# qwopqwop200/GPTQ-for-LLaMa

Measured on NVIDIA H100. Metric: tokens/sec LLaMA-7B int4 g128 batch=1; matvec HBM GB/s vs 3.35 TB/s roofline, higher is better.
Workload: dtype f16

## Files before the change

### gptq-for-llama_b200/csrc/decode_mega.cu

```cuda
#include <cuda.h>
#include <cudaTypedefs.h>

#include "common.cuh"
#include "int4_core.cuh"
#include "kernels.h"

namespace gptq {
namespace {

using namespace int4;

constexpr int kTeams = 2;
constexpr int kTeamWarps = 8;
constexpr int kTeamThreads = kTeamWarps * 32;
constexpr int kConsumers = kTeams * kTeamThreads;
constexpr int kConsumerWarps = kTeams * kTeamWarps;
constexpr int kBlock = kConsumers + 32 * kTeams;
constexpr int kSlabCols = 256;
constexpr int kStageSteps = 4;
constexpr int kStepBytes = 4096;
constexpr int kScaleOff = kStageSteps * kStepBytes;
constexpr int kZeroOff = kScaleOff + 512;
constexpr int kStageBytes = 17 * 1024;
constexpr int kHD = 128;
// ... 33 lines not shown
    const int optr_s0 = (ring).stages
#define OPTRACE_END(ring, layer, op)                                                                                   \
    do {                                                                                                               \
        if (g_mega_trace != nullptr && threadIdx.x == 0 && (layer) == 2) {                                              \
            g_mega_trace[blockIdx.x * 64 + 48 + 3 * (op)] = (unsigned long long)(clock64() - optr_t0);                  \
            g_mega_trace[blockIdx.x * 64 + 48 + 3 * (op) + 1] = (unsigned long long)((ring).waited - optr_w0);          \
            g_mega_trace[blockIdx.x * 64 + 48 + 3 * (op) + 2] = (unsigned long long)((ring).stages - optr_s0);          \
        }                                                                                                              \
    } while (0)
#else
#define OPTRACE_BEGIN(ring) \
    do {                    \
    } while (0)
#define OPTRACE_END(ring, layer, op) \
    do {                             \
    } while (0)
#endif

struct MatDesc {
    const __half* sc;
    const uint32_t* qz;
    int gs_steps;
    int tmap;
    int chunk0;
};
struct LayerDesc {
    MatDesc qkv, o, gate, up, down;
    const __half* input_norm;
    const __half* post_norm;
    const int32_t* qkv_perm;
    const int32_t* o_perm;
    const int32_t* mlp_perm;
};
constexpr int kMaxTP = 8;
struct MegaParams {
    int n_layers, H, Hq, I, V, v0, v1, n_heads, max_seq, n_stages, lm_rows;
    int tp_size, tp_rank, tp_exchange;
    float eps, inv_base, scale;
    const __half* embed;
    const __half* final_norm;
    const __half* lm_head;
    const int32_t* tokens;
    const int32_t* positions;
    __half* k_cache;
    __half* v_cache;
    size_t layer_stride;
    __half* logits;
    int32_t* next_token;
    __half* resid[2];
    float* acc_qkv;
    float* acc_o;
    float* acc_g;
    float* acc_u;
    float* acc_d;
    float* part;
    float* rope_cs;
    unsigned long long* bar;
    float* acc_o_loc;
    float* acc_d_loc;
    float* acc_o_peer[kMaxTP];
    float* acc_d_peer[kMaxTP];
    __half* logits_peer[kMaxTP];
    unsigned long long* xbar_peer[kMaxTP];
    LayerDesc layers[kMaxLayers];
    CUtensorMap tmaps[6];
    int batch, xs_stride;
};

__device__ __forceinline__ void team_range(unsigned T, unsigned U, unsigned nb, int& a, int& b) {
    a = (int)((T * U) / nb);
    b = (int)(((T + 1) * U) / nb);
}
struct HeadTeams {
    int first, count;
};
__device__ __forceinline__ HeadTeams head_teams(int head, int n_heads, unsigned nb) {
    const int base = (int)nb / n_heads, rem = (int)nb % n_heads;
    HeadTeams h;
    h.first = head * base + min(head, rem);
    h.count = base + (head < rem ? 1 : 0);
    return h;
}
__device__ __forceinline__ void attn_range(unsigned T, int n_heads, unsigned nb, int upb, int& head, int& b0, int& b1) {
    const int base = (int)nb / n_heads, rem = (int)nb % n_heads;
    const int split = rem * (base + 1);
    int idx, cnt;
    if ((int)T < split) {
        head = (int)T / (base + 1);
        idx = (int)T - head * (base + 1);
        cnt = base + 1;
    } else {
        head = rem + ((int)T - split) / base;
        idx = ((int)T - split) % base;
        cnt = base;
    }
    b0 = idx * upb / cnt;
    b1 = (idx + 1) * upb / cnt;
}

__device__ __forceinline__ int stage_steps(int gpos, int gs_steps, int left) { return min(min(kStageSteps, gs_steps - gpos), left); }

__device__ __forceinline__ int step_pos(const MegaParams& p, int s) { return min(max(p.positions[s], 0), p.max_seq - 1); }

__device__ __forceinline__ HeadTeams seq_teams(const MegaParams& p, int s, unsigned nb) {
    int before = 0, mine = 0, tot = 0;
#pragma unroll 1
    for (int i = 0; i < p.batch; ++i) {
        const int units = step_pos(p, i) / kKeysPerUnit + 1;
        before += i < s ? units : 0;
        mine = i == s ? units : mine;
        tot += units;
    }
    const long long extra = (long long)nb - (long long)p.batch * p.n_heads;
    HeadTeams h;
    h.first = s * p.n_heads + (int)(extra * before / tot);
    h.count = (s + 1) * p.n_heads + (int)(extra * (before + mine) / tot) - h.first;
    return h;
}
__device__ __forceinline__ int team_seq(const MegaParams& p, unsigned T, unsigned nb, HeadTeams& st) {
    int s = 0;
#pragma unroll 1
    for (;; ++s) {
        st = seq_teams(p, s, nb);
        if ((int)T < st.first + st.count || s == p.batch - 1) return s;
    }
}
template <bool BATCH>
__device__ __forceinline__ int attn_work(const MegaParams& p, unsigned T, unsigned nb, int& pos, int& Tlen, int& head, int& b0, int& b1) {
    int s = 0;
    HeadTeams st{0, (int)nb};
    if constexpr (BATCH) s = team_seq(p, T, nb, st);
    pos = step_pos(p, s);
    Tlen = pos + 1;
    const int upb = (Tlen + kKeysPerUnit - 1) / kKeysPerUnit;
    attn_range(T - st.first, p.n_heads, st.count, upb, head, b0, b1);
    return s;
}

__device__ __forceinline__ void team_sync(int team) { asm volatile("bar.sync %0, 256;" ::"r"(team + 1) : "memory"); }
__device__ __forceinline__ void cta_sync() { asm volatile("bar.sync 3, 512;" ::: "memory"); }

struct ProdRing {
    uint32_t ring, full, empty;
    int stage, use, nstages;
#ifdef GPTQ_TRACE
    long long blocked;
#endif
};
__device__ __forceinline__ uint32_t prod_acquire(ProdRing& r, uint32_t& bar) {
#ifdef GPTQ_TRACE
    const long long t0 = clock64();
#endif
    if (r.use > 0) mbar_wait_backoff(r.empty + r.stage * 8, (r.use - 1) & 1u);
#ifdef GPTQ_TRACE
    r.blocked += clock64() - t0;
#endif
    bar = r.full + r.stage * 8;
    return r.ring + r.stage * kStageBytes;
}
__device__ __forceinline__ void prod_advance(ProdRing& r) {
    if (++r.stage == r.nstages) {
        r.stage = 0;
        ++r.use;
    }
}

__device__ __forceinline__ void tma_load_3d(uint32_t dst, const CUtensorMap* tm, int c0, int c1, int c2, uint32_t bar, uint64_t policy) {
    asm volatile("cp.async.bulk.tensor.3d.shared::cluster.global.mbarrier::complete_tx::bytes.L2::cache_hint [%0], [%1, {%2, %3, %4}], [%5], %6;" ::"r"(dst),
                 "l"(tm), "r"(c0), "r"(c1), "r"(c2), "r"(bar), "l"(policy)
                 : "memory");
}

struct StageLoad {
    const CUtensorMap* tm;
    int row, chunk, n;
    const void* a;
    const void* b;
    uint32_t a_off, b_off, a_bytes, b_bytes;
};

template <bool BATCH>
struct StageWalk {
    enum { kQ, kA, kO, kG, kD, kL, kEnd };
    int l = 0, op = -1, u = 0, u1 = 0;
    int Tlen = 0;
    size_t kv = 0;

    __device__ __forceinline__ bool next(const MegaParams& p, unsigned T, unsigned nb, StageLoad& s) {
        while (u >= u1) {
            if (op == kEnd) return false;
            if (++op == kL && l + 1 < p.n_layers) {
                ++l;
                op = kQ;
            }
            if (op == kA) {
                int pos, head;
                const int seq = attn_work<BATCH>(p, T, nb, pos, Tlen, head, u, u1);
                kv = (size_t)l * p.layer_stride + (size_t)(seq * p.n_heads + head) * p.max_seq * kHD;
            } else if (op == kL) {
                team_range(T, (unsigned)((p.v1 - p.v0 + p.lm_rows - 1) / p.lm_rows), nb, u, u1);
            } else if (op != kEnd) {
                int K, N, nm;
                matvec_shape(p, K, N, nm);
                team_range(T, (unsigned)(nm * (N / kSlabCols)) * (K / 32), nb, u, u1);
            }
        }
        s.tm = nullptr;
        s.b = nullptr;
        s.b_bytes = 0;
        if (op == kA) {
            const int nrows = min(kKeysPerUnit, Tlen - u * kKeysPerUnit);
            const size_t off = kv + (size_t)u * kKeysPerUnit * kHD;
            s.a = p.k_cache + off;
            s.b = p.v_cache + off;
            s.a_off = 0;
            s.b_off = kVOff;
            s.a_bytes = s.b_bytes = nrows * 256;
            ++u;
        } else if (op == kL) {
            const int R = p.lm_rows, nrows = min(R, p.v1 - p.v0 - u * R);
            s.a = p.lm_head + (size_t)u * R * p.H;
            s.a_off = 0;
            s.a_bytes = (uint32_t)nrows * p.H * 2;
            ++u;
        } else {
            int K, N, nm;
            matvec_shape(p, K, N, nm);
            const int nk = K / 32, nslab = N / kSlabCols;
            const int slab_v = u / nk, ks = u - slab_v * nk;
            const int mi = slab_v >= nslab ? 1 : 0, slab = slab_v - mi * nslab;
            const LayerDesc& L = p.layers[l];
            const MatDesc& m = op == kQ ? L.qkv : op == kO ? L.o : op == kD ? L.down : mi ? L.up : L.gate;
            const int g = ks / m.gs_steps;
            s.n = stage_steps(ks - g * m.gs_steps, m.gs_steps, min(nk - ks, u1 - u));
            s.tm = &p.tmaps[(s.n == kStageSteps ? 0 : 3) + m.tmap];
            s.row = ks * 4;
            s.chunk = m.chunk0 + slab * (kSlabCols / 32);
            s.a = m.sc + (size_t)g * N + slab * kSlabCols;
            s.b = m.qz + (size_t)g * (N >> 3) + slab * (kSlabCols / 8);
            s.a_off = kScaleOff;
            s.b_off = kZeroOff;
            s.a_bytes = 512;
            s.b_bytes = 128;
            u += s.n;
        }
        return true;
    }

    __device__ __forceinline__ void matvec_shape(const MegaParams& p, int& K, int& N, int& nm) const {
        K = op == kO ? p.Hq : op == kD ? p.I : p.H;
        N = op == kQ ? 3 * p.Hq : op == kG ? p.I : p.H;
        nm = op == kG ? 2 : 1;
    }
};

template <bool BATCH>
__device__ void producer_loop(const MegaParams& p, ProdRing r, unsigned T, unsigned nb) {
    uint64_t policy;
    asm volatile("createpolicy.fractional.L2::evict_first.b64 %0, 1.0;" : "=l"(policy));
    StageWalk<BATCH> walk;
    StageLoad s;
#pragma unroll 1
    while (walk.next(p, T, nb, s)) {
        uint32_t bar;
        const uint32_t dst = prod_acquire(r, bar);
        mbar_expect_tx(bar, (s.tm != nullptr ? s.n * kStepBytes : 0) + s.a_bytes + s.b_bytes);
        if (s.tm != nullptr) {
            if (s.n == kStageSteps) {
                tma_load_3d(dst, s.tm, 0, s.row, s.chunk, bar, policy);
            } else {
                for (int j = 0; j < s.n; ++j) tma_load_3d(dst + j * kStepBytes, s.tm, 0, s.row + 4 * j, s.chunk, bar, policy);
            }
        }
        bulk_copy_g2s(dst + s.a_off, s.a, s.a_bytes, bar, policy);
        if (s.b != nullptr) bulk_copy_g2s(dst + s.b_off, s.b, s.b_bytes, bar, policy);
        prod_advance(r);
    }
#ifdef GPTQ_TRACE
    if (g_mega_trace != nullptr && (T & 1) == 0) g_mega_trace[(T / kTeams) * 64 + 63] = (unsigned long long)r.blocked;
#endif
}

struct ConsRing {
    uint32_t ring, full;
    uint32_t tile, bar;
    uint32_t parity;
    int left, nstages;
#ifdef GPTQ_TRACE
    long long waited;
    int stages;
#endif
};
__device__ __forceinline__ uint32_t cons_wait(ConsRing& c) {
#ifdef GPTQ_TRACE
    const long long t0 = clock64();
#endif
    mbar_wait(c.bar, c.parity);
#ifdef GPTQ_TRACE
    c.waited += clock64() - t0;
    ++c.stages;
#endif
    return c.tile;
}
__device__ __forceinline__ void cons_release(ConsRing& c, int lane) {
    __syncwarp();
    if (lane == 0) mbar_arrive(c.bar + kMaxStages * 8);
    c.tile += kStageBytes;
    c.bar += 8;
    if (--c.left == 0) {
        c.left = c.nstages;
        c.tile = c.ring;
        c.bar = c.full;
        c.parity ^= 1u;
    }
}

__device__ __forceinline__ void grid_barrier(unsigned long long* bar, unsigned long long& target) {
    cta_sync();
    if (threadIdx.x == 0) {
        target += gridDim.x;
        asm volatile("red.release.gpu.global.add.u64 [%0], 1;" ::"l"(bar) : "memory");
        unsigned long long v;
        do {
            asm volatile("ld.acquire.gpu.global.u64 %0, [%1];" : "=l"(v) : "l"(bar) : "memory");
        } while (v < target);
    }
    cta_sync();
}

__device__ __forceinline__ void tp_barrier(const MegaParams& p, unsigned long long& target) {
    cta_sync();
    if (threadIdx.x == 0) {
        target += gridDim.x;
        asm volatile("fence.acq_rel.sys;" ::: "memory");
        for (int q = 0; q < p.tp_size; ++q)
            asm volatile("red.relaxed.sys.global.add.u64 [%0], 1;" ::"l"(p.xbar_peer[q] + 32 * p.tp_rank) : "memory");
        const unsigned long long* mine = p.xbar_peer[p.tp_rank];
        for (int q = 0; q < p.tp_size; ++q) {
            unsigned long long v;
            do {
                asm volatile("ld.relaxed.sys.global.u64 %0, [%1];" : "=l"(v) : "l"(mine + 32 * q) : "memory");
            } while (v < target);
        }
        asm volatile("fence.acq_rel.gpu;" ::: "memory");
    }
    cta_sync();
}

__device__ __forceinline__ void tp_exchange(const MegaParams& p, float* loc, float* const* peers, int n) {
    const int per = (n + gridDim.x - 1) / gridDim.x;
    const int lo = blockIdx.x * per, hi = min(n, lo + per);
    for (int j = lo + threadIdx.x; j < hi; j += kConsumers) {
        const float v = ld_cg(loc + j);
        loc[j] = 0.f;
        for (int q = 0; q < p.tp_size; ++q) asm volatile("red.relaxed.sys.global.add.f32 [%0], %1;" ::"l"(peers[q] + j), "f"(v) : "memory");
    }
}

__device__ __forceinline__ void zero_slice(float* buf, int n) {
    const int per = ((n / 4 + gridDim.x - 1) / gridDim.x);
    const int lo = blockIdx.x * per, hi = min(n / 4, lo + per);
    for (int i = lo + threadIdx.x; i < hi; i += kConsumers) reinterpret_cast<float4*>(buf)[i] = make_float4(0.f, 0.f, 0.f, 0.f);
}

__device__ __forceinline__ float block_sum(float v, uint32_t& m, float* red_s) {
    v = warp_sum(v);
    const uint32_t mx = __reduce_max_sync(0xffffffffu, m & 0xffffu), my = __reduce_max_sync(0xffffffffu, m >> 16);
    cta_sync();
    if ((threadIdx.x & 31) == 0) {
        red_s[threadIdx.x >> 5] = v;
        reinterpret_cast<uint32_t*>(red_s)[kConsumerWarps + (threadIdx.x >> 5)] = mx | (my << 16);
    }
    cta_sync();
    float t = 0.f;
    m = 0;
#pragma unroll
    for (int w = 0; w < kConsumerWarps; ++w) {
        t += red_s[w];
        m = __vmaxu2(m, reinterpret_cast<const uint32_t*>(red_s)[kConsumerWarps + w]);
    }
    return t;
}

__device__ __forceinline__ uint4 perm8(uint32_t w0, uint32_t w1, uint32_t w2, uint32_t w3) {
    return make_uint4(__byte_perm(w0, w2, 0x5410), __byte_perm(w0, w2, 0x7632), __byte_perm(w1, w3, 0x5410), __byte_perm(w1, w3, 0x7632));
}
__device__ __forceinline__ int perm_pos(int j) { return ((j & 3) << 1) + (j >> 2); }

struct XScale {
    float even, odd, inv;
};
__device__ __forceinline__ XScale x_scale(float m) {
    const int e = min(max(14 - ((int)((__float_as_uint(m) >> 23) & 255u) - 127), -1), 38);
    return XScale{__int_as_float((127 + e) << 23), __int_as_float((123 + e) << 23), __int_as_float((127 - e) << 23)};
}
__device__ __forceinline__ uint32_t max_abs8(uint32_t m, uint4 v) {
    m = __vmaxu2(m, v.x & 0x7fff7fffu);
    m = __vmaxu2(m, v.y & 0x7fff7fffu);
    m = __vmaxu2(m, v.z & 0x7fff7fffu);
    return __vmaxu2(m, v.w & 0x7fff7fffu);
}
__device__ __forceinline__ uint32_t scale_h2(uint32_t w, float f) {
    const float2 v = __half22float2(u32_as_h2(w));
    return h2_as_u32(__floats2half2_rn(v.x * f, v.y * f));
}
__device__ __forceinline__ uint4 scale_run(uint4 v, const XScale& sc) {
    return make_uint4(scale_h2(v.x, sc.even), scale_h2(v.y, sc.odd), scale_h2(v.z, sc.even), scale_h2(v.w, sc.odd));
}

__device__ __forceinline__ float run_sum(uint4 v) {
    const float2 a = __half22float2(u32_as_h2(v.x)), b = __half22float2(u32_as_h2(v.y)), c = __half22float2(u32_as_h2(v.z)), d = __half22float2(u32_as_h2(v.w));
    const float even = (a.x + a.y) + (c.x + c.y), odd = (b.x + b.y) + (d.x + d.y);
    return fmaf(odd, 16.0f, even);
}
__device__ __forceinline__ void scale_and_sum(__half* xs, int nsteps, float* xsum, const XScale& sc, int tid, int nthreads) {
    const int n4 = nsteps * 4;
    for (int base = 0; base < n4; base += nthreads) {
        const int idx = base + tid;
        float v = 0.f;
        if (idx < n4) {
            uint4* run = reinterpret_cast<uint4*>(xs + idx * 8);
            const uint4 r = scale_run(*run, sc);
            *run = r;
            v = run_sum(r);
        }
        v += __shfl_xor_sync(0xffffffffu, v, 1);
        v += __shfl_xor_sync(0xffffffffu, v, 2);
        if (idx < n4 && (idx & 3) == 0) xsum[idx >> 2] = v;
    }
}

template <bool ACT, bool PLAIN>
__device__ void stage_norm(const MegaParams& p, const __half* src, const float* acc, const __half* norm_w, __half* resid_out, __half* xs, float* xsum,
                           float* xinv, __half* tmp, float* red_s, const int32_t* perm) {
    const int H = p.H, tid = threadIdx.x, nch = H / 8;
    float ss = 0.f;
    uint32_t xm = 0, wm = 0;
    uint4 nwv[2];
#pragma unroll
    for (int i = 0; i < 2; ++i) {
        const int c = tid + i * kConsumers;
        nwv[i] = make_uint4(0, 0, 0, 0);
        if (c < nch) {
            nwv[i] = *reinterpret_cast<const uint4*>(norm_w + c * 8);
            const uint4 v = ld_cg_u4(src + c * 8);
            uint32_t xv[4] = {v.x, v.y, v.z, v.w};
            if (acc != nullptr) {
                const float4 a0 = ld_cg4(acc + c * 8), a1 = ld_cg4(acc + c * 8 + 4);
                const float av[8] = {a0.x, a0.y, a0.z, a0.w, a1.x, a1.y, a1.z, a1.w};
#pragma unroll
                for (int j = 0; j < 4; ++j)
                    xv[j] = h2_as_u32(__hadd2(u32_as_h2(xv[j]), __floats2half2_rn(av[2 * j], av[2 * j + 1])));
            }
#pragma unroll
            for (int j = 0; j < 4; ++j) {
                const float2 f = __half22float2(u32_as_h2(xv[j]));
                ss = fmaf(f.x, f.x, ss);
                ss = fmaf(f.y, f.y, ss);
            }
            const uint4 xq = make_uint4(xv[0], xv[1], xv[2], xv[3]);
            *reinterpret_cast<uint4*>(tmp + c * 8) = xq;
            xm = max_abs8(xm, xq);
            wm = max_abs8(wm, nwv[i]);
        }
    }
    uint32_t m = max(xm & 0xffffu, xm >> 16) | (max(wm & 0xffffu, wm >> 16) << 16);
    const float tot = block_sum(ss, m, red_s);
    const float rstd = 1.0f / sqrtf(tot / (float)H + p.eps);
    XScale sc{1.f, 1.f, 1.f};
    if constexpr (!PLAIN) {
        sc = x_scale(__half2float(__ushort_as_half((unsigned short)(m & 0xffffu))) * rstd * __half2float(__ushort_as_half((unsigned short)(m >> 16))) * 1.001f);
        if (tid == 0) *xinv = sc.inv;
    }
    if (resid_out != nullptr) {
        const int per = (nch + gridDim.x - 1) / gridDim.x;
        const int c = blockIdx.x * per + tid;
        if (tid < per && c < nch) *reinterpret_cast<uint4*>(resid_out + c * 8) = *reinterpret_cast<const uint4*>(tmp + c * 8);
    }
#pragma unroll
    for (int i = 0; i < 2; ++i) {
        const int c = tid + i * kConsumers;
        if (c < nch) {
            float xf[8];
            bool gathered = false;
            if constexpr (ACT) {
                if (perm != nullptr) {
                    const ::int4 p0 = *reinterpret_cast<const ::int4*>(perm + c * 8), p1 = *reinterpret_cast<const ::int4*>(perm + c * 8 + 4);
                    const int k[8] = {p0.x, p0.y, p0.z, p0.w, p1.x, p1.y, p1.z, p1.w};
#pragma unroll
                    for (int j = 0; j < 8; ++j) xf[j] = __half2float(tmp[k[j]]);
                    gathered = true;
                }
            }
            if (!gathered) {
                const uint4 v = *reinterpret_cast<const uint4*>(tmp + c * 8);
                const uint32_t xv[4] = {v.x, v.y, v.z, v.w};
#pragma unroll
                for (int j = 0; j < 4; ++j) {
                    const float2 f = __half22float2(u32_as_h2(xv[j]));
                    xf[2 * j] = f.x;
                    xf[2 * j + 1] = f.y;
                }
            }
            const uint32_t wv[4] = {nwv[i].x, nwv[i].y, nwv[i].z, nwv[i].w};
            uint32_t o[4];
#pragma unroll
            for (int j = 0; j < 4; ++j) {
                const float2 wf = __half22float2(u32_as_h2(wv[j]));
                o[j] = h2_as_u32(__floats2half2_rn(__fmul_rn(__fmul_rn(xf[2 * j], rstd), wf.x), __fmul_rn(__fmul_rn(xf[2 * j + 1], rstd), wf.y)));
            }
            if constexpr (PLAIN) {
                *reinterpret_cast<uint4*>(xs + c * 8) = make_uint4(o[0], o[1], o[2], o[3]);
            } else {
                const uint4 pv = scale_run(perm8(o[0], o[1], o[2], o[3]), sc);
                *reinterpret_cast<uint4*>(xs + c * 8) = pv;
                float v = run_sum(pv);
                v += __shfl_xor_sync(0xffffffffu, v, 1);
                v += __shfl_xor_sync(0xffffffffu, v, 2);
                if ((c & 3) == 0) xsum[c >> 2] = v;
            }
        }
    }
    cta_sync();
}

__device__ __forceinline__ void mma_16816_z(float (&d)[4], uint32_t a0, uint32_t a1, uint32_t a2, uint32_t a3, uint32_t b0, uint32_t b1) {
    asm volatile("mma.sync.aligned.m16n8k16.row.col.f32.f16.f16.f32 {%0,%1,%2,%3}, {%4,%5,%6,%7}, {%8,%9}, {%10,%10,%10,%10};"
                 : "=f"(d[0]), "=f"(d[1]), "=f"(d[2]), "=f"(d[3])
                 : "r"(a0), "r"(a1), "r"(a2), "r"(a3), "r"(b0), "r"(b1), "f"(0.f));
}

__device__ __forceinline__ void nibble_regs(uint32_t q, uint32_t (&a)[4]) {
    const uint32_t q8 = q >> 8;
    a[0] = q & 0x000f000fu;
    a[1] = q & 0x00f000f0u;
    a[2] = q8 & 0x000f000fu;
    a[3] = q8 & 0x00f000f0u;
}

template <bool FIRST>
__device__ __forceinline__ void step_mma(const uint4& q, const uint4& xf, float (&acc0)[4], float (&acc1)[4]) {
    uint32_t c0[4], c1[4], c2[4], c3[4];
    nibble_regs(q.x, c0);
    nibble_regs(q.y, c1);
    nibble_regs(q.z, c2);
    nibble_regs(q.w, c3);
    if (FIRST) {
        mma_16816_z(acc0, c0[0], c1[0], c0[1], c1[1], xf.x, xf.y);
        mma_16816_z(acc1, c2[0], c3[0], c2[1], c3[1], xf.x, xf.y);
    } else {
        mma_16816(acc0, c0[0], c1[0], c0[1], c1[1], xf.x, xf.y);
        mma_16816(acc1, c2[0], c3[0], c2[1], c3[1], xf.x, xf.y);
    }
    mma_16816(acc0, c0[2], c1[2], c0[3], c1[3], xf.z, xf.w);
    mma_16816(acc1, c2[2], c3[2], c2[3], c3[3], xf.z, xf.w);
}

enum XMode { X_FULL = 0, X_ATTN = 1, X_SWIGLU = 2 };

struct TeamCtx {
    int team, wt, lane, ttid;
    unsigned T, nb;
    __half* xseg;
    float* xsum_seg;
    float* xinv_seg;
    uint32_t* xmax;
    uint8_t* scratch;
};

template <int NB>
__device__ __forceinline__ float merge_records(const MegaParams& p, const HeadTeams& ht, int d) {
    float M = -INFINITY, Ls = 0.f, O = 0.f;
#pragma unroll 1
    for (int ib = 0; ib < ht.count; ib += NB) {
        float mv[NB], lv[NB], ov[NB];
#pragma unroll
        for (int i = 0; i < NB; ++i) {
            const bool on = ib + i < ht.count;
            const float* rc = p.part + (size_t)(ht.first + (on ? ib + i : 0)) * kRec;
            const float m = ld_cg(rc), l = ld_cg(rc + 1), o = ld_cg(rc + 4 + d);
            mv[i] = on ? m : -INFINITY;
            lv[i] = on ? l : 0.f;
            ov[i] = on ? o : 0.f;
        }
        float Mb = M;
#pragma unroll
        for (int i = 0; i < NB; ++i) Mb = fmaxf(Mb, mv[i]);
        const float w0 = (M == -INFINITY) ? 0.f : expf(M - Mb);
        Ls *= w0;
        O *= w0;
#pragma unroll
        for (int i = 0; i < NB; ++i) {
            const float w = (mv[i] == -INFINITY) ? 0.f : expf(mv[i] - Mb);
            Ls = fmaf(lv[i], w, Ls);
            O = fmaf(ov[i], w, O);
        }
        M = Mb;
    }
    return O / Ls;
}

template <int XMODE, bool ACT, bool BATCH>
__device__ void stage_range(const MegaParams& p, const TeamCtx& tc, int nk, int u0, int u1, const int32_t* perm) {
    const int nun = u1 - u0, nfeat = nun * 32;
    const int nbat = BATCH ? p.batch : 1;
    const int ksb = u0 % nk;
    auto k_of = [&](int e) {
        int ks = ksb + (e >> 5);
        if (ks >= nk) ks -= nk;
        return ks * 32 + (e & 31);
    };
    if (tc.ttid < nbat) tc.xmax[tc.ttid] = 0;
    team_sync(tc.team);
    if constexpr (XMODE == X_SWIGLU) {
        for (int c = tc.ttid; c < nun * 4 * nbat; c += kTeamThreads) {
            int s = 0, cs = c;
            if constexpr (BATCH) {
                s = c / (nun * 4);
                cs = c - s * (nun * 4);
            }
            const int k = k_of(cs * 8);
            const float* ag = p.acc_g + (size_t)s * p.I + k;
            const float* au = p.acc_u + (size_t)s * p.I + k;
            const float4 g0 = ld_cg4(ag), g1 = ld_cg4(ag + 4);
            const float4 a0 = ld_cg4(au), a1 = ld_cg4(au + 4);
            const uint32_t o0 = h2_as_u32(__floats2half2_rn(swiglu(g0.x, a0.x), swiglu(g0.y, a0.y)));
            const uint32_t o1 = h2_as_u32(__floats2half2_rn(swiglu(g0.z, a0.z), swiglu(g0.w, a0.w)));
            const uint32_t o2 = h2_as_u32(__floats2half2_rn(swiglu(g1.x, a1.x), swiglu(g1.y, a1.y)));
            const uint32_t o3 = h2_as_u32(__floats2half2_rn(swiglu(g1.z, a1.z), swiglu(g1.w, a1.w)));
            const uint4 pv = perm8(o0, o1, o2, o3);
            *reinterpret_cast<uint4*>(tc.xseg + (size_t)s * p.xs_stride + cs * 8) = pv;
            const uint32_t m = max_abs8(0, pv);
            atomicMax(tc.xmax + s, max(m & 0xffffu, m >> 16));
        }
    } else {
        constexpr int kBatch = 12;
        uint32_t vmax = 0;
        auto put = [&](__half* xseg, int e, float v) {
            const __half hv = __float2half_rn(v);
            xseg[(e & ~7) + perm_pos(e & 7)] = hv;
            vmax = max(vmax, (uint32_t)(__half_as_ushort(hv) & 0x7fffu));
        };
        bool fast = false;
        if constexpr (!BATCH) {
            const int nA = min(nun, nk - ksb);
            const int hA0 = (ksb * 32) / kHD, hA1 = ((ksb + nA) * 32 - 1) / kHD;
            const int nslotA = hA1 - hA0 + 1, nslotB = (nun > nA) ? ((nun - nA) * 32 - 1) / kHD + 1 : 0;
            fast = (nslotA + nslotB <= kTeamWarps) && (nun <= nk) && ((int)tc.nb / p.n_heads + 1 <= kBatch);
            if constexpr (ACT) fast = fast && (perm == nullptr);
            if (fast) {
                float* wts = reinterpret_cast<float*>(tc.scratch);
                float ov[kBatch];
                int slot = 0;
                auto fetch = [&](int e) {
                    const bool active = e < nfeat;
                    const int k = k_of(active ? e : 0);
                    const int head = k / kHD, d = k - head * kHD;
                    slot = ((e >> 5) < nA) ? head - hA0 : nslotA + head;
                    const HeadTeams ht = head_teams(head, p.n_heads, tc.nb);
#pragma unroll
                    for (int i = 0; i < kBatch; ++i) ov[i] = (active && i < ht.count) ? ld_cg(p.part + (size_t)(ht.first + i) * kRec + 4 + d) : 0.f;
                };
                auto emit = [&](int e) {
                    if (e < nfeat) {
                        float O = 0.f;
#pragma unroll
                        for (int i = 0; i < kBatch; ++i) O = fmaf(wts[slot * kBatch + i], ov[i], O);
                        put(tc.xseg, e, O);
                    }
                };
                fetch(tc.ttid);
                if (tc.wt < nslotA + nslotB) {
                    const int lane = tc.lane;
                    const int head = tc.wt < nslotA ? hA0 + tc.wt : tc.wt - nslotA;
                    const HeadTeams ht = head_teams(head, p.n_heads, tc.nb);
                    float m = -INFINITY, l = 0.f;
                    if (lane < ht.count) {
                        m = ld_cg(p.part + (size_t)(ht.first + lane) * kRec);
                        l = ld_cg(p.part + (size_t)(ht.first + lane) * kRec + 1);
                    }
                    float M = m;
#pragma unroll
                    for (int o = 8; o > 0; o >>= 1) M = fmaxf(M, __shfl_xor_sync(0xffffffffu, M, o));
                    M = __shfl_sync(0xffffffffu, M, 0);
                    const float w = (m == -INFINITY) ? 0.f : expf(m - M);
                    float L = l * w;
#pragma unroll
                    for (int o = 8; o > 0; o >>= 1) L += __shfl_xor_sync(0xffffffffu, L, o);
                    L = __shfl_sync(0xffffffffu, L, 0);
                    if (lane < kBatch) wts[tc.wt * kBatch + lane] = w / L;
                }
                team_sync(tc.team);
                emit(tc.ttid);
                for (int e = tc.ttid + kTeamThreads; e - tc.ttid < nfeat; e += kTeamThreads) {
                    fetch(e);
                    emit(e);
                }
                atomicMax(tc.xmax, vmax);
            }
        }
        if (!fast) {
            for (int s = 0; s < nbat; ++s) {
                HeadTeams st{0, (int)tc.nb};
                if constexpr (BATCH) st = seq_teams(p, s, tc.nb);
                for (int e = tc.ttid; e < nfeat; e += kTeamThreads) {
                    int k = k_of(e);
                    if constexpr (ACT) {
                        if (perm != nullptr) k = perm[k];
                    }
                    const int head = k / kHD, d = k - head * kHD;
                    HeadTeams ht = head_teams(head, p.n_heads, st.count);
                    ht.first += st.first;
                    put(tc.xseg + (size_t)s * p.xs_stride, e, merge_records<kBatch>(p, ht, d));
                }
                atomicMax(tc.xmax + s, vmax);
                vmax = 0;
            }
        }
    }
    team_sync(tc.team);
    for (int s = 0; s < nbat; ++s) {
        const XScale sc = x_scale(__half2float(__ushort_as_half((unsigned short)tc.xmax[s])));
        if (tc.ttid == 0) tc.xinv_seg[s] = sc.inv;
        scale_and_sum(tc.xseg + (size_t)s * p.xs_stride, nun, tc.xsum_seg + s * (p.H / 32), sc, tc.ttid, kTeamThreads);
    }
    team_sync(tc.team);
}

template <int NM, int XMODE, bool ACT = false, bool BATCH = false>
__device__ void run_matvec(const MegaParams& p, ConsRing& ring, const TeamCtx& tc, int gs_steps, int K, int N, float* out0, float* out1, const __half* xs_full,
                           const float* xsum_full, const float* xinv_full, const int32_t* perm = nullptr, float* const* peers = nullptr) {
    const int lane = tc.lane, g = lane >> 2, t = lane & 3;
    const int nk = K / 32, nslab = N / kSlabCols;
    int u, u_end;
    team_range(tc.T, (unsigned)(NM * nslab) * nk, tc.nb, u, u_end);
    const int cg = (g >> 1) | ((g & 1) << 2);
    const int col_l = 4 * cg + t;
    const uint32_t lane_a0 = (uint32_t)((tc.wt * 16 + t) * 128 + ((cg ^ t) * 16));
    const uint32_t lane_a1 = (uint32_t)((tc.wt * 16 + t) * 128 + ((cg ^ t ^ 4) * 16));
    const uint32_t lane_b = (uint32_t)((tc.wt * 4 + t) * 128 + ((cg ^ (4 * (tc.wt & 1) + t)) * 16));
    const uint32_t lane_s = (uint32_t)(kScaleOff + (tc.wt * 32 + col_l) * 2);
    const uint32_t lane_z = (uint32_t)(kZeroOff + (tc.wt * 4 + (cg >> 1)) * 4);
    const int zshift = (cg & 1) * 16 + t * 4;
    const float unit = 16777216.0f;
    const int B = p.batch;
    const int xsum_hi = BATCH ? (min(2 * t + 1, B - 1) - min(2 * t, B - 1)) * (p.H / 32) : 0;
    const int u_begin = u;
    if constexpr (XMODE != X_FULL) {
        if (u < u_end) {
#ifdef GPTQ_TRACE
            const long long stg0 = clock64();
#endif
            stage_range<XMODE, ACT, BATCH>(p, tc, nk, u, u_end, perm);
#ifdef GPTQ_TRACE
            if (g_mega_trace != nullptr && threadIdx.x == 0) g_mega_trace[blockIdx.x * 64 + 36 + XMODE] += (unsigned long long)(clock64() - stg0);
#endif
        }
    }

#pragma unroll 1
    while (u < u_end) {
        const int slab_v = u / nk;
        const int ks0 = u - slab_v * nk;
        const int nseg = min(nk - ks0, u_end - u);
        const int mi = (NM > 1 && slab_v >= nslab) ? 1 : 0;
        float* outp = (mi ? out1 : out0) + (slab_v - mi * nslab) * kSlabCols + tc.wt * 32 + col_l;

        uint32_t xaddr;
        const float* xsum;
        if constexpr (XMODE == X_FULL) {
            xaddr = smem_u32(xs_full) + (ks0 * 32 + t * 8) * 2;
            xsum = xsum_full + ks0;
        } else {
            xaddr = smem_u32(tc.xseg) + ((u - u_begin) * 32 + t * 8) * 2;
            xsum = tc.xsum_seg + (u - u_begin);
        }
        float totb[4][2];
        if constexpr (BATCH) {
            xaddr += (uint32_t)(min(g, B - 1) * p.xs_stride * 2);
            xsum += min(2 * t, B - 1) * (p.H / 32);
#pragma unroll
            for (int i = 0; i < 4; ++i) totb[i][0] = totb[i][1] = 0.f;
        }

        float tot = 0.f;
        int left = nseg, gpos = ks0 % gs_steps;
#pragma unroll 1
        while (left > 0) {
            const int n = stage_steps(gpos, gs_steps, left);
            const uint32_t st = cons_wait(ring);
            float acc0[4], acc1[4];
            float xs4, xs4b;
            if (n == kStageSteps) {
                uint4 q[4], xf[4];
#pragma unroll
                for (int j = 0; j < 4; ++j) q[j] = lds128(st + j * 512 + ((j & 1) ? lane_a1 : lane_a0));
#pragma unroll
                for (int j = 0; j < 4; ++j) xf[j] = lds128(xaddr + j * 64);
                step_mma<true>(q[0], xf[0], acc0, acc1);
                step_mma<false>(q[1], xf[1], acc0, acc1);
                step_mma<false>(q[2], xf[2], acc0, acc1);
                step_mma<false>(q[3], xf[3], acc0, acc1);
                xs4 = (xsum[0] + xsum[1]) + (xsum[2] + xsum[3]);
                if constexpr (BATCH) xs4b = (xsum[xsum_hi] + xsum[xsum_hi + 1]) + (xsum[xsum_hi + 2] + xsum[xsum_hi + 3]);
            } else {
                {
                    const uint4 q = lds128(st + lane_b), xf = lds128(xaddr);
                    step_mma<true>(q, xf, acc0, acc1);
                    xs4 = xsum[0];
                    if constexpr (BATCH) xs4b = xsum[xsum_hi];
                }
#pragma unroll 1
                for (int j = 1; j < n; ++j) {
                    const uint4 q = lds128(st + lane_b + j * kStepBytes), xf = lds128(xaddr + j * 64);
                    step_mma<false>(q, xf, acc0, acc1);
                    xs4 += xsum[j];
                    if constexpr (BATCH) xs4b += xsum[xsum_hi + j];
                }
            }
            if constexpr (BATCH) {
                uint32_t s01, s23, zw;
                asm volatile("ld.shared.v2.u32 {%0, %1}, [%2];" : "=r"(s01), "=r"(s23) : "r"(st + (uint32_t)(kScaleOff + (tc.wt * 32 + 4 * cg) * 2)));
                asm volatile("ld.shared.u32 %0, [%1];" : "=r"(zw) : "r"(st + lane_z));
                const float2 sa = __half22float2(u32_as_h2(s01)), sb = __half22float2(u32_as_h2(s23));
                const float sc[4] = {sa.x, sa.y, sb.x, sb.y};
                const float av[4][2] = {{acc0[0], acc0[1]}, {acc0[2], acc0[3]}, {acc1[0], acc1[1]}, {acc1[2], acc1[3]}};
#pragma unroll
                for (int i = 0; i < 4; ++i) {
                    const float z = (float)(((zw >> ((cg & 1) * 16 + 4 * i)) & 15u) + 1u);
                    totb[i][0] = fmaf(sc[i], fmaf(av[i][0], unit, -z * xs4), totb[i][0]);
                    totb[i][1] = fmaf(sc[i], fmaf(av[i][1], unit, -z * xs4b), totb[i][1]);
                }
            } else {
                uint32_t sh, zw;
                asm volatile("ld.shared.u16 %0, [%1];" : "=r"(sh) : "r"(st + lane_s));
                asm volatile("ld.shared.u32 %0, [%1];" : "=r"(zw) : "r"(st + lane_z));
                const float a = (t & 2) ? ((t & 1) ? acc1[2] : acc1[0]) : ((t & 1) ? acc0[2] : acc0[0]);
                const float z = (float)(((zw >> zshift) & 15u) + 1u);
                tot = fmaf(__half2float(__ushort_as_half((unsigned short)sh)), fmaf(a, unit, -z * xs4), tot);
            }
            cons_release(ring, lane);
            xaddr += n * 64;
            xsum += n;
            left -= n;
            gpos += n;
            if (gpos == gs_steps) gpos = 0;
        }
        const float* xinv = XMODE == X_FULL ? xinv_full : tc.xinv_seg;
        if constexpr (BATCH) {
            float* outq = (mi ? out1 : out0) + (slab_v - mi * nslab) * kSlabCols + tc.wt * 32 + 4 * cg;
#pragma unroll
            for (int j = 0; j < 2; ++j) {
                const float inv = xinv[min(2 * t + j, B - 1)];
                if (2 * t + j < B)
                    asm volatile("red.global.add.v4.f32 [%0], {%1, %2, %3, %4};" ::"l"(outq + (size_t)(2 * t + j) * N), "f"(totb[0][j] * inv), "f"(totb[1][j] * inv),
                                 "f"(totb[2][j] * inv), "f"(totb[3][j] * inv)
                                 : "memory");
            }
        } else {
            tot *= xinv[0];
            if (peers == nullptr) {
                asm volatile("red.global.add.f32 [%0], %1;" ::"l"(outp), "f"(tot) : "memory");
            } else {
                const size_t off = (size_t)(outp - out0);
                for (int q = 0; q < p.tp_size; ++q) asm volatile("red.relaxed.sys.global.add.f32 [%0], %1;" ::"l"(peers[q] + off), "f"(tot) : "memory");
            }
        }
        u += nseg;
    }
}

template <bool BATCH>
__device__ void run_attention(const MegaParams& p, ConsRing& ring, const TeamCtx& tc, int layer) {
    int pos, Tlen, head, b0, b_end;
    const int seq = attn_work<BATCH>(p, tc.T, tc.nb, pos, Tlen, head, b0, b_end);
    float* red_o = reinterpret_cast<float*>(tc.scratch);
    float* red_ml = reinterpret_cast<float*>(tc.scratch + 4096);
    float* q_s = reinterpret_cast<float*>(tc.scratch);
    __half* knew = reinterpret_cast<__half*>(tc.scratch + 512);
    __half* vnew = knew + kHD;
    const int ttid = tc.ttid, lane = tc.lane, grp = ttid >> 3, j = ttid & 7;
    const int ub_new = pos / kKeysPerUnit;
    __half* kc_l = p.k_cache + layer * p.layer_stride;
    __half* vc_l = p.v_cache + layer * p.layer_stride;
    float* rec = p.part + (size_t)tc.T * kRec;
    if (b0 >= b_end) {
        if (ttid < kHD) rec[4 + ttid] = 0.f;
        if (ttid == 0) {
            rec[0] = -INFINITY;
            rec[1] = 0.f;
        }
        return;
    }
    {
        const int nseg = b_end - b0;
        const bool owns_new = (ub_new >= b0 && ub_new < b_end);
        team_sync(tc.team);
        if (ttid < kHD) {
            const int i = ttid & 63;
            const bool hi = ttid >= 64;
            const float c = ld_cg(p.rope_cs + seq * kHD + i), s = ld_cg(p.rope_cs + seq * kHD + 64 + i);
            const float* aq = p.acc_qkv + (size_t)seq * 3 * p.Hq + head * kHD;
            const float qx = __half2float(__float2half_rn(ld_cg(aq + i))), qy = __half2float(__float2half_rn(ld_cg(aq + i + 64)));
            const float qr = hi ? __fadd_rn(__fmul_rn(qx, s), __fmul_rn(qy, c)) : __fsub_rn(__fmul_rn(qx, c), __fmul_rn(qy, s));
            q_s[ttid] = __half2float(__float2half_rn(qr));
            if (owns_new) {
                const float* ak = aq + p.Hq;
                const float* av = aq + 2 * p.Hq;
                const float kx = __half2float(__float2half_rn(ld_cg(ak + i))), ky = __half2float(__float2half_rn(ld_cg(ak + i + 64)));
                const float kr = hi ? __fadd_rn(__fmul_rn(kx, s), __fmul_rn(ky, c)) : __fsub_rn(__fmul_rn(kx, c), __fmul_rn(ky, s));
                const __half kh = __float2half_rn(kr), vh = __float2half_rn(ld_cg(av + ttid));
                knew[ttid] = kh;
                vnew[ttid] = vh;
                const size_t off = ((size_t)(seq * p.n_heads + head) * p.max_seq + pos) * kHD + ttid;
                kc_l[off] = kh;
                vc_l[off] = vh;
            }
        }
        team_sync(tc.team);
        float qr[16];
#pragma unroll
        for (int d = 0; d < 8; ++d) {
            qr[d] = q_s[8 * j + d];
            qr[8 + d] = q_s[64 + 8 * j + d];
        }
        float mloc = -INFINITY, lloc = 0.f, o[16];
#pragma unroll
        for (int d = 0; d < 16; ++d) o[d] = 0.f;
#pragma unroll 1
        for (int b = b0; b < b0 + nseg; ++b) {
            const uint32_t st = cons_wait(ring);
            if (b == ub_new) {
                team_sync(tc.team);
                const int row = pos - b * kKeysPerUnit;
                if (ttid < 16) {
                    sts128(st + row * 256 + ttid * 16, reinterpret_cast<const uint4*>(knew)[ttid]);
                    fence_proxy_async_smem();
                } else if (ttid < 32) {
                    sts128(st + kVOff + row * 256 + (ttid - 16) * 16, reinterpret_cast<const uint4*>(vnew)[ttid - 16]);
                    fence_proxy_async_smem();
                }
                team_sync(tc.team);
            }
            const int key = b * kKeysPerUnit + grp;
            const bool valid = key < Tlen;
            float s = 0.f;
            if (valid) {
                const uint4 k0 = lds128(st + grp * 256 + j * 16), k1 = lds128(st + grp * 256 + 128 + j * 16);
                const uint32_t w[8] = {k0.x, k0.y, k0.z, k0.w, k1.x, k1.y, k1.z, k1.w};
#pragma unroll
                for (int e = 0; e < 8; ++e) {
                    const float2 f = __half22float2(u32_as_h2(w[e]));
                    s = fmaf(qr[2 * e], f.x, s);
                    s = fmaf(qr[2 * e + 1], f.y, s);
                }
            }
            s += __shfl_xor_sync(0xffffffffu, s, 1);
            s += __shfl_xor_sync(0xffffffffu, s, 2);
            s += __shfl_xor_sync(0xffffffffu, s, 4);
            if (valid) {
                s *= p.scale;
                const float mnew = fmaxf(mloc, s);
                const float alpha = (mloc == -INFINITY) ? 0.f : expf(mloc - mnew);
                const float pw = expf(s - mnew);
                lloc = fmaf(lloc, alpha, pw);
                const uint4 v0 = lds128(st + kVOff + grp * 256 + j * 16), v1 = lds128(st + kVOff + grp * 256 + 128 + j * 16);
                const uint32_t w[8] = {v0.x, v0.y, v0.z, v0.w, v1.x, v1.y, v1.z, v1.w};
#pragma unroll
                for (int e = 0; e < 8; ++e) {
                    const float2 f = __half22float2(u32_as_h2(w[e]));
                    o[2 * e] = fmaf(o[2 * e], alpha, pw * f.x);
                    o[2 * e + 1] = fmaf(o[2 * e + 1], alpha, pw * f.y);
                }
                mloc = mnew;
            }
            cons_release(ring, lane);
        }
        team_sync(tc.team);
#pragma unroll
        for (int sh = 8; sh <= 16; sh <<= 1) {
            const float mo = __shfl_xor_sync(0xffffffffu, mloc, sh), lo = __shfl_xor_sync(0xffffffffu, lloc, sh);
            const float mn = fmaxf(mloc, mo);
            const float wa = (mloc == -INFINITY) ? 0.f : expf(mloc - mn), wb = (mo == -INFINITY) ? 0.f : expf(mo - mn);
            lloc = lloc * wa + lo * wb;
#pragma unroll
            for (int d = 0; d < 16; ++d) {
                const float oo = __shfl_xor_sync(0xffffffffu, o[d], sh);
                o[d] = o[d] * wa + oo * wb;
            }
            mloc = mn;
        }
        if (lane < 8) {
            if (lane == 0) {
                red_ml[tc.wt * 2] = mloc;
                red_ml[tc.wt * 2 + 1] = lloc;
            }
#pragma unroll
            for (int d = 0; d < 8; ++d) {
                red_o[tc.wt * kHD + 8 * lane + d] = o[d];
                red_o[tc.wt * kHD + 64 + 8 * lane + d] = o[8 + d];
            }
        }
        team_sync(tc.team);
        if (ttid < kHD) {
            float M = -INFINITY;
#pragma unroll
            for (int w = 0; w < kTeamWarps; ++w) M = fmaxf(M, red_ml[w * 2]);
            float L = 0.f, O = 0.f;
#pragma unroll
            for (int w = 0; w < kTeamWarps; ++w) {
                const float mw = red_ml[w * 2];
                const float wgt = (mw == -INFINITY) ? 0.f : expf(mw - M);
                L = fmaf(red_ml[w * 2 + 1], wgt, L);
                O = fmaf(red_o[w * kHD + ttid], wgt, O);
            }
            rec[4 + ttid] = O;
            if (ttid == 0) {
                rec[0] = M;
                rec[1] = L;
            }
        }
    }
}

__device__ void run_lm_head(const MegaParams& p, ConsRing& ring, const TeamCtx& tc, const __half* xs_plain) {
    const int R = p.lm_rows, H = p.H, nch = H / 8;
    int u, u_end;
    const int nloc = p.v1 - p.v0;
    team_range(tc.T, (unsigned)((nloc + R - 1) / R), tc.nb, u, u_end);
    float* part_s = reinterpret_cast<float*>(tc.scratch);
    float xr[4][8];
#pragma unroll
    for (int i = 0; i < 4; ++i) {
        const int c = tc.ttid + i * kTeamThreads;
        if (c < nch) {
            const uint4 v = *reinterpret_cast<const uint4*>(xs_plain + c * 8);
            const uint32_t w[4] = {v.x, v.y, v.z, v.w};
#pragma unroll
            for (int e = 0; e < 4; ++e) {
                const float2 f = __half22float2(u32_as_h2(w[e]));
                xr[i][2 * e] = f.x;
                xr[i][2 * e + 1] = f.y;
            }
        } else {
#pragma unroll
            for (int e = 0; e < 8; ++e) xr[i][e] = 0.f;
        }
    }
    int buf = 0;
#pragma unroll 1
    for (; u < u_end; ++u) {
        const int nrows = min(R, nloc - u * R);
        const uint32_t st = cons_wait(ring);
        float* ps = part_s + buf * (R * kTeamWarps);
#pragma unroll 1
        for (int r = 0; r < nrows; ++r) {
            float a = 0.f;
#pragma unroll
            for (int i = 0; i < 4; ++i) {
                const int c = tc.ttid + i * kTeamThreads;
                if (c < nch) {
                    const uint4 wv = lds128(st + (uint32_t)(r * H * 2 + c * 16));
                    const uint32_t w[4] = {wv.x, wv.y, wv.z, wv.w};
#pragma unroll
                    for (int e = 0; e < 4; ++e) {
                        const float2 f = __half22float2(u32_as_h2(w[e]));
                        a = fmaf(f.x, xr[i][2 * e], a);
                        a = fmaf(f.y, xr[i][2 * e + 1], a);
                    }
                }
            }
            a = warp_sum(a);
            if (tc.lane == 0) ps[r * kTeamWarps + tc.wt] = a;
        }
        cons_release(ring, tc.lane);
        team_sync(tc.team);
        if (tc.ttid < nrows) {
            float a = 0.f;
#pragma unroll
            for (int w = 0; w < kTeamWarps; ++w) a += ps[tc.ttid * kTeamWarps + w];
            const __half lg = __float2half_rn(a);
            for (int q = 0; q < p.tp_size; ++q) p.logits_peer[q][(size_t)p.v0 + (size_t)u * R + tc.ttid] = lg;
        }
        buf ^= 1;
    }
}

__device__ void run_lm_head_batch(const MegaParams& p, ConsRing& ring, const TeamCtx& tc, const __half* xs_plain) {
    const int R = p.lm_rows, H = p.H, nch = H / 8, B = p.batch;
    int u, u_end;
    team_range(tc.T, (unsigned)((p.V + R - 1) / R), tc.nb, u, u_end);
    float* part_s = reinterpret_cast<float*>(tc.scratch);
    const uint32_t xbase = smem_u32(xs_plain);
    int buf = 0;
#pragma unroll 1
    for (; u < u_end; ++u) {
        const int nrows = min(R, p.V - u * R);
        const uint32_t st = cons_wait(ring);
        float* ps = part_s + buf * (R * B * kTeamWarps);
#pragma unroll 1
        for (int r = 0; r < nrows; ++r) {
            float a[kMaxBatch];
#pragma unroll
            for (int s = 0; s < kMaxBatch; ++s) a[s] = 0.f;
#pragma unroll 1
            for (int c = tc.ttid; c < nch; c += kTeamThreads) {
                const uint4 wv = lds128(st + (uint32_t)(r * H * 2 + c * 16));
                const uint32_t w[4] = {wv.x, wv.y, wv.z, wv.w};
#pragma unroll
                for (int s = 0; s < kMaxBatch; ++s) {
                    if (s < B) {
                        const uint4 xv = lds128(xbase + (uint32_t)((s * p.xs_stride + c * 8) * 2));
                        const uint32_t x[4] = {xv.x, xv.y, xv.z, xv.w};
#pragma unroll
                        for (int e = 0; e < 4; ++e) {
                            const float2 f = __half22float2(u32_as_h2(w[e])), xf = __half22float2(u32_as_h2(x[e]));
                            a[s] = fmaf(f.x, xf.x, a[s]);
                            a[s] = fmaf(f.y, xf.y, a[s]);
                        }
                    }
                }
            }
#pragma unroll
            for (int s = 0; s < kMaxBatch; ++s) {
                if (s < B) {
                    const float v = warp_sum(a[s]);
                    if (tc.lane == 0) ps[(r * B + s) * kTeamWarps + tc.wt] = v;
                }
            }
        }
        cons_release(ring, tc.lane);
        team_sync(tc.team);
        if (tc.ttid < nrows * B) {
            const int r = tc.ttid / B, s = tc.ttid - r * B;
            float a = 0.f;
#pragma unroll
            for (int w = 0; w < kTeamWarps; ++w) a += ps[tc.ttid * kTeamWarps + w];
            p.logits[(size_t)s * p.V + (size_t)u * R + r] = __float2half_rn(a);
        }
        buf ^= 1;
    }
}

__device__ __forceinline__ void argmax_row(const __half* row, int V, int32_t* out) {
    const int tid = threadIdx.x, warp = tid >> 5, lane = tid & 31;
    float best = -INFINITY;
    int idx = 0x7fffffff;
    for (int i = tid; i < V; i += kConsumers) {
        const float v = __half2float(ld_cg_h(row + i));
// ... 480 lines not shown
```

Before: 446.4.

## Consume two ring stages per iteration and interleave their MMA chains

In the non-batched consumer loop, the code now waits on two consecutive full stages at once. It interleaves the two independent MMA accumulation chains to raise instruction-level parallelism and releases both stages before applying the dequant epilogue. Scale and zero loads are hoisted ahead of the MMAs, and the release is moved before the epilogue math in the single-stage path too, so producers can refill sooner. The cost is higher register pressure, and waiting for the second stage can add latency when the ring is shallow.

```diff
diff --git a/gptq-for-llama_b200/csrc/decode_mega.cu b/gptq-for-llama_b200/csrc/decode_mega.cu
--- a/gptq-for-llama_b200/csrc/decode_mega.cu
+++ b/gptq-for-llama_b200/csrc/decode_mega.cu
@@ -359,6 +359,20 @@
 #endif
     return c.tile;
 }
+__device__ __forceinline__ uint32_t cons_wait2(ConsRing& c) {
+    cons_wait(c);
+    const bool wrap = c.left == 1;
+    ConsRing n = c;
+    n.tile = wrap ? c.ring : c.tile + kStageBytes;
+    n.bar = wrap ? c.full : c.bar + 8;
+    n.parity = wrap ? c.parity ^ 1u : c.parity;
+    const uint32_t st = cons_wait(n);
+#ifdef GPTQ_TRACE
+    c.waited = n.waited;
+    c.stages = n.stages;
+#endif
+    return st;
+}
 __device__ __forceinline__ void cons_release(ConsRing& c, int lane) {
     __syncwarp();
     if (lane == 0) mbar_arrive(c.bar + kMaxStages * 8);
@@ -612,6 +626,11 @@
     mma_16816(acc0, c0[2], c1[2], c0[3], c1[3], xf.z, xf.w);
     mma_16816(acc1, c2[2], c3[2], c2[3], c3[3], xf.z, xf.w);
 }
+
+struct StageEpi {
+    uint32_t s0, s1, zw;
+    float xs4, xs4b;
+};
 
 enum XMode { X_FULL = 0, X_ATTN = 1, X_SWIGLU = 2 };
 
@@ -841,13 +860,80 @@
         }
 
         float tot = 0.f;
+        auto load_epi = [&](uint32_t st, const float* xs, int n) {
+            StageEpi e;
+            if constexpr (BATCH) {
+                asm volatile("ld.shared.v2.u32 {%0, %1}, [%2];" : "=r"(e.s0), "=r"(e.s1) : "r"(st + (uint32_t)(kScaleOff + (tc.wt * 32 + 4 * cg) * 2)));
+            } else {
+                asm volatile("ld.shared.u16 %0, [%1];" : "=r"(e.s0) : "r"(st + lane_s));
+            }
+            asm volatile("ld.shared.u32 %0, [%1];" : "=r"(e.zw) : "r"(st + lane_z));
+            if (n == kStageSteps) {
+                e.xs4 = (xs[0] + xs[1]) + (xs[2] + xs[3]);
+                if constexpr (BATCH) e.xs4b = (xs[xsum_hi] + xs[xsum_hi + 1]) + (xs[xsum_hi + 2] + xs[xsum_hi + 3]);
+            } else {
+                e.xs4 = xs[0];
+                if constexpr (BATCH) e.xs4b = xs[xsum_hi];
+#pragma unroll 1
+                for (int j = 1; j < n; ++j) {
+                    e.xs4 += xs[j];
+                    if constexpr (BATCH) e.xs4b += xs[xsum_hi + j];
+                }
+            }
+            return e;
+        };
+        auto apply_epi = [&](const StageEpi& e, const float (&acc0)[4], const float (&acc1)[4]) {
+            if constexpr (BATCH) {
+                const float2 sa = __half22float2(u32_as_h2(e.s0)), sb = __half22float2(u32_as_h2(e.s1));
+                const float sc[4] = {sa.x, sa.y, sb.x, sb.y};
+                const float av[4][2] = {{acc0[0], acc0[1]}, {acc0[2], acc0[3]}, {acc1[0], acc1[1]}, {acc1[2], acc1[3]}};
+#pragma unroll
+                for (int i = 0; i < 4; ++i) {
+                    const float z = (float)(((e.zw >> ((cg & 1) * 16 + 4 * i)) & 15u) + 1u);
+                    totb[i][0] = fmaf(sc[i], fmaf(av[i][0], unit, -z * e.xs4), totb[i][0]);
+                    totb[i][1] = fmaf(sc[i], fmaf(av[i][1], unit, -z * e.xs4b), totb[i][1]);
+                }
+            } else {
+                const float a = (t & 2) ? ((t & 1) ? acc1[2] : acc1[0]) : ((t & 1) ? acc0[2] : acc0[0]);
+                const float z = (float)(((e.zw >> zshift) & 15u) + 1u);
+                tot = fmaf(__half2float(__ushort_as_half((unsigned short)e.s0)), fmaf(a, unit, -z * e.xs4), tot);
+            }
+        };
         int left = nseg, gpos = ks0 % gs_steps;
 #pragma unroll 1
         while (left > 0) {
             const int n = stage_steps(gpos, gs_steps, left);
+            const int gpos2 = gpos + n == gs_steps ? 0 : gpos + n;
+            if (!BATCH && n == kStageSteps && left > kStageSteps && stage_steps(gpos2, gs_steps, left - kStageSteps) == kStageSteps) {
+                const uint32_t sb = cons_wait2(ring), sa = ring.tile;
+                const StageEpi ea = load_epi(sa, xsum, kStageSteps), eb = load_epi(sb, xsum + kStageSteps, kStageSteps);
+                float a0[4], a1[4], b0[4], b1[4];
+#pragma unroll
+                for (int j = 0; j < kStageSteps; ++j) {
+                    const uint32_t lo = (j & 1) ? lane_a1 : lane_a0;
+                    const uint4 qa = lds128(sa + j * 512 + lo), xa = lds128(xaddr + j * 64);
+                    const uint4 qb = lds128(sb + j * 512 + lo), xb = lds128(xaddr + (kStageSteps + j) * 64);
+                    if (j == 0) {
+                        step_mma<true>(qa, xa, a0, a1);
+                        step_mma<true>(qb, xb, b0, b1);
+                    } else {
+                        step_mma<false>(qa, xa, a0, a1);
+                        step_mma<false>(qb, xb, b0, b1);
+                    }
+                }
+                cons_release(ring, lane);
+                cons_release(ring, lane);
+                apply_epi(ea, a0, a1);
+                apply_epi(eb, b0, b1);
+                xaddr += 2 * kStageSteps * 64;
+                xsum += 2 * kStageSteps;
+                left -= 2 * kStageSteps;
+                gpos = gpos2 + kStageSteps == gs_steps ? 0 : gpos2 + kStageSteps;
+                continue;
+            }
             const uint32_t st = cons_wait(ring);
+            const StageEpi e = load_epi(st, xsum, n);
             float acc0[4], acc1[4];
-            float xs4, xs4b;
             if (n == kStageSteps) {
                 uint4 q[4], xf[4];
 #pragma unroll
@@ -858,50 +944,23 @@
                 step_mma<false>(q[1], xf[1], acc0, acc1);
                 step_mma<false>(q[2], xf[2], acc0, acc1);
                 step_mma<false>(q[3], xf[3], acc0, acc1);
-                xs4 = (xsum[0] + xsum[1]) + (xsum[2] + xsum[3]);
-                if constexpr (BATCH) xs4b = (xsum[xsum_hi] + xsum[xsum_hi + 1]) + (xsum[xsum_hi + 2] + xsum[xsum_hi + 3]);
             } else {
                 {
                     const uint4 q = lds128(st + lane_b), xf = lds128(xaddr);
                     step_mma<true>(q, xf, acc0, acc1);
-                    xs4 = xsum[0];
-                    if constexpr (BATCH) xs4b = xsum[xsum_hi];
                 }
 #pragma unroll 1
                 for (int j = 1; j < n; ++j) {
                     const uint4 q = lds128(st + lane_b + j * kStepBytes), xf = lds128(xaddr + j * 64);
                     step_mma<false>(q, xf, acc0, acc1);
-                    xs4 += xsum[j];
-                    if constexpr (BATCH) xs4b += xsum[xsum_hi + j];
                 }
             }
-            if constexpr (BATCH) {
-                uint32_t s01, s23, zw;
-                asm volatile("ld.shared.v2.u32 {%0, %1}, [%2];" : "=r"(s01), "=r"(s23) : "r"(st + (uint32_t)(kScaleOff + (tc.wt * 32 + 4 * cg) * 2)));
-                asm volatile("ld.shared.u32 %0, [%1];" : "=r"(zw) : "r"(st + lane_z));
-                const float2 sa = __half22float2(u32_as_h2(s01)), sb = __half22float2(u32_as_h2(s23));
-                const float sc[4] = {sa.x, sa.y, sb.x, sb.y};
-                const float av[4][2] = {{acc0[0], acc0[1]}, {acc0[2], acc0[3]}, {acc1[0], acc1[1]}, {acc1[2], acc1[3]}};
-#pragma unroll
-                for (int i = 0; i < 4; ++i) {
-                    const float z = (float)(((zw >> ((cg & 1) * 16 + 4 * i)) & 15u) + 1u);
-                    totb[i][0] = fmaf(sc[i], fmaf(av[i][0], unit, -z * xs4), totb[i][0]);
-                    totb[i][1] = fmaf(sc[i], fmaf(av[i][1], unit, -z * xs4b), totb[i][1]);
-                }
-            } else {
-                uint32_t sh, zw;
-                asm volatile("ld.shared.u16 %0, [%1];" : "=r"(sh) : "r"(st + lane_s));
-                asm volatile("ld.shared.u32 %0, [%1];" : "=r"(zw) : "r"(st + lane_z));
-                const float a = (t & 2) ? ((t & 1) ? acc1[2] : acc1[0]) : ((t & 1) ? acc0[2] : acc0[0]);
-                const float z = (float)(((zw >> zshift) & 15u) + 1u);
-                tot = fmaf(__half2float(__ushort_as_half((unsigned short)sh)), fmaf(a, unit, -z * xs4), tot);
-            }
             cons_release(ring, lane);
+            apply_epi(e, acc0, acc1);
             xaddr += n * 64;
             xsum += n;
             left -= n;
-            gpos += n;
-            if (gpos == gs_steps) gpos = 0;
+            gpos = gpos2;
         }
         const float* xinv = XMODE == X_FULL ? xinv_full : tc.xinv_seg;
         if constexpr (BATCH) {
```

After: 455.2, median of 6. +2.0%, better.
